# PeterouZh/CIPS-3D

Hardware: AMD Instinct MI355X
Metric: rendered imgs/sec (G fwd+bwd) (higher is better)
Workload: dtype f32 (dense layers as 3-pass split-operand MFMA with fp32 accumulate: SIREN forward on fp16 hi/lo planes, ~2e-7 rel., sigma in the fp32 class; INR head and all backward GEMMs on bf16 hi/lo planes, ~5e-6 rel. per layer; everything else fp32); 1 GPU; FFHQ r64, 24 SIREN evals/ray (num_steps 24, hierarchical False), batch 32/GPU, G fwd+bwd, all 9 CIPS blocks; global_batch=32, parallelism=dp1, rccl_ranks=0, inr_gemm_mode=bf16x3, launch=hipGraph replay, grad_reduce=none

## Files before the change

### cips3d_amd/_lib.py

```python
import ctypes as C
import os

_HERE = os.path.dirname(os.path.abspath(__file__))
LIB_PATH = os.path.join(_HERE, "lib", "libcips3d_hip.so")

vp = C.c_void_p
i32 = C.c_int
i64 = C.c_longlong
f32 = C.c_float


class SirenWeights(C.Structure):
    _fields_ = [(n, vp) for n in
                ("w0", "b0", "w1", "b1", "ws", "bs", "wc", "bc", "wf", "bf",
                 "g0", "p0", "g1", "p1", "gc", "pc")] + [("box_scale", f32), ("trig_mode", i32)]


class SirenGrads(C.Structure):
    _fields_ = [(n, vp) for n in ("dg0", "dp0", "dg1", "dp1", "dgc", "dpc", "dw0", "db0", "dw1", "db1", "dws", "dbs", "dwc",
                                  "dbc", "dwf", "dbf")]


class RayParams(C.Structure):
    _fields_ = [("xg", vp), ("yg", vp), ("zg", vp), ("cam2world", vp), ("jitter", vp), ("zvals", vp), ("zc", f32), ("H", i32),
# ... 120 lines not shown
    "cips_live_points": (i32, [vp, i32, i32, vp, vp, vp]),
    "cips_composite_has_dead_samples": (i32, [i32]),
    "cips_live_points_clamp": (i32, [vp, vp, f32, i32, i32, i32, i32, i32, vp, vp, vp]),
    "cips_composite_bwd_listed": (i32, [vp, vp, vp, vp, f32, vp, vp, vp, i32, i32, i32, i32, vp]),
    "cips_march_fwd_x3_geo": (i32, [C.POINTER(SirenWeights), C.POINTER(RayParams), vp, f32, i32, i32, vp, vp, vp, vp, vp, vp, i32, vp, vp, vp, vp]),
    "cips_composite_fwd_geo": (i32, [vp, vp, vp, vp, vp, vp, vp, f32, vp, vp, vp, vp, vp, i32, i32, i32, i32, vp, vp, vp, vp]),
    "cips_composite_bwd_geo": (i32, [vp, vp, vp, vp, vp, vp, vp, f32, vp, vp, vp, vp, vp, vp, i32, i32, i32, i32, vp, vp, vp, vp]),
    "cips_composite_bwd_live_geo": (i32, [vp, vp, vp, vp, vp, vp, vp, f32, vp, vp, vp, vp, vp, vp, vp, vp, i32, i32, i32, i32, vp, vp, vp, vp]),
    "cips_composite_bwd_listed_geo": (i32, [vp, vp, vp, vp, f32, vp, vp, vp, i32, i32, i32, i32, vp, vp, vp]),
    "cips_gemm_f32": (i32, [C.POINTER(GemmDesc), vp]),
    "cips_gemm_bf16x3": (i32, [C.POINTER(GemmX3Desc), vp]),
    "cips_gemm_bf16x3_fuses_torgb": (i32, [C.POINTER(GemmX3Desc)]),
    "cips_gemm_bf16x3_takes_addp": (i32, [C.POINTER(GemmX3Desc)]),
    "cips_gemm_bf16x3_takes_bkmajor": (i32, [C.POINTER(GemmX3Desc)]),
    "cips_torgb_finish": (i32, [vp, i32, vp, vp, i64, i32, vp]),
    "cips_equal_linear_scratch": (i64, [i32, i32, i32, i32]),
    "cips_equal_linear": (i32, [i32, vp, vp, vp, f32, f32, vp, vp, i32, i32, i32, vp]),
    "cips_gemm_bf16x3_km": (i32, [C.POINTER(GemmX3Desc), vp]),
    "cips_gemm_bf16x3_km_grouped": (i32, [C.POINTER(GemmX3Desc), i32, vp]),
    "cips_gemm_bf16": (i32, [C.POINTER(GemmX3Desc), vp]),
    "cips_gemm_bf16_fuses_torgb": (i32, [C.POINTER(GemmX3Desc)]),
    "cips_gemm_bf16_takes_addp": (i32, [C.POINTER(GemmX3Desc)]),
    "cips_gemm_bf16_km": (i32, [C.POINTER(GemmX3Desc), vp]),
    "cips_gemm_bf16_km_grouped": (i32, [C.POINTER(GemmX3Desc), i32, vp]),
    "cips_lrelu_bwd_bias_slices": (i32, [i32]),
    "cips_lrelu_bwd_bias": (i32, [vp, vp, vp, vp, i64, i32, f32, f32, vp]),
    "cips_lrelu_bwd_bias_finish": (i32, [vp, vp, i32, i32, i32, vp]),
    "cips_lrelu_bwd_bias_nhwc_tiles": (i32, [i32]),
    "cips_lrelu_bwd_bias_nhwc": (i32, [vp, vp, vp, vp, vp, i32, i32, i32, f32, f32, vp]),
    "cips_conv1x1_smallk": (i32, [vp, vp, vp, i32, i32, i32, i32, vp]),
# ... 8 lines not shown
    "cips_conv_weight_prep_max_jobs": (i32, []),
    "cips_conv_weight_prep_batch": (i32, [C.POINTER(WPrepJob), i32, vp]),
    "cips_conv2d_x3_dgrad_s2": (i32, [C.POINTER(ConvDgradS2Desc), vp]),
    "cips_conv_wgrad_finish": (i32, [vp, vp, i32, i32, i32, i32, f32, vp]),
    "cips_conv2d_bf16": (i32, [C.POINTER(ConvX3Desc), vp]),
    "cips_conv2d_bf16_ksplit": (i32, [i32, i32, i32, i32]),
    "cips_conv2d_bf16_dgrad_s2": (i32, [C.POINTER(ConvDgradS2Desc), vp]),
    "cips_conv2d_bf16_wgrad": (i32, [C.POINTER(ConvWgradDesc), vp]),
    "cips_modfc_prep_x3": (i32, [vp, vp, vp, vp, vp, vp, vp, i32, i32, i32, f32, vp]),
    "cips_torgb_fwd_x3": (i32, [vp, vp, vp, vp, vp, i64, i32, i32, vp]),
    "cips_torgb_bwd_w_x3": (i32, [vp, vp, vp, vp, vp, vp, i64, i32, vp]),
    "cips_modfc_prep": (i32, [vp, vp, vp, vp, vp, i32, i32, i32, f32, vp]),
    "cips_modfc_prep_bwd": (i32, [vp, vp, vp, vp, vp, vp, vp, i32, i32, i32, vp]),
    "cips_modfc_max_jobs": (i32, []),
    "cips_modfc_prep_x3_batch": (i32, [C.POINTER(ModfcPrepJob), i32, i32, C.c_float, vp]),
    "cips_modfc_prep_bwd_batch": (i32, [C.POINTER(ModfcBwdJob), i32, i32, vp]),
    "cips_modfc_prep_x3_batch_form": (i32, [C.POINTER(ModfcPrepJob), i32, i32]),
    "cips_modfc_prep_bwd_batch_form": (i32, [C.POINTER(ModfcBwdJob), i32, i32]),
    "cips_modfc_prep_bwd_batch_cores": (i32, [C.POINTER(ModfcBwdJob), i32, i32, vp]),
    "cips_cores_colsum_parts": (i32, []),
    "cips_opt_chunk": (i32, []),
    "cips_opt_step": (i32, [vp, vp, vp, i32, vp, vp, f32, f32, f32, f32, f32, f32, i32, vp, vp]),
    "cips_pyramid_loss_scratch": (i64, [i32, i32, i32, i32, i32]),
    "cips_pyramid_loss_fwd": (i32, [vp, vp, vp, C.POINTER(C.c_double), i32, i32, C.c_double, vp, vp, vp, i64, i32, i32, i32, i32, vp]),
    "cips_pyramid_loss_bwd": (i32, [vp, vp, vp, i32, i64, vp]),
    "cips_reproject_fwd": (i32, [vp, vp, vp, vp, f32, f32, f32, vp, vp, vp, i32, i32, i32, i32, i32, i32, vp]),
    "cips_reproject_bwd": (i32, [vp, vp, vp, vp, vp, f32, f32, vp, vp, i32, i32, i32, i32, i32, i32, vp]),
    "cips_raster_fwd": (i32, [vp] * 5 + [f32, f32, f32, i32] + [vp] * 4 + [i64] + [vp] * 4 + [i32] * 5 + [vp]),
    "cips_raster_interp": (i32, [vp] * 4 + [f32, vp] + [i32] * 6 + [vp]),
    "cips_volume_bake": (i32, [vp] * 4 + [i32] * 4 + [vp]),
# ... 5 lines not shown
    "cips_volume_render_bwd_cam": (i32, [vp] * 8 + [f32, i32, i32] + [vp] * 5 + [i32] * 8 + [vp]),
    "cips_camera_pose": (i32, [vp, vp, i32, f32, f32, f32, f32, vp, vp, vp, i32, vp]),
    "cips_grouped_linear_max_jobs": (i32, []),
    "cips_grouped_linear_fwd": (i32, [C.POINTER(GlinJob), i32, i32, vp]),
    "cips_grouped_linear_scratch": (i64, [C.POINTER(GlinJob), i32, i32]),
    "cips_grouped_linear_bwd": (i32, [C.POINTER(GlinJob), i32, i32, vp, vp, i64, vp]),
    "cips_rownorm_fwd": (i32, [vp, vp, vp, vp, vp, i32, i32, i32, f32, vp]),
    "cips_rownorm_bwd": (i32, [vp] * 9 + [i32, i32, i32, f32, vp]),
    "cips_torgb_fwd": (i32, [vp, vp, vp, vp, i64, i32, i32, vp]),
    "cips_torgb_bwd_partials": (i32, [i64]),
    "cips_torgb_bwd_w": (i32, [vp, vp, vp, vp, vp, i64, i32, vp]),
    "cips_torgb_bwd_x": (i32, [vp, vp, vp, vp, f32, vp, vp, i64, i32, vp]),
    "cips_torgb_bwd_w_x3_batch": (i32, [vp, vp, i32, vp, vp, vp, vp, i64, i32, vp]),
    "cips_torgb_bwd_w_x3_batch_cores": (i32, [vp, vp, i32, vp, vp, vp, vp, i64, i32, vp]),
    "cips_torgb_bwd_x_x3": (i32, [vp, vp, vp, f32, vp, vp, vp, i64, i32, vp]),
    "cips_fused_bias_act": (i32, [vp, vp, vp, vp, i64, i32, i32, i32, i32, f32, f32, vp]),
    "cips_diffaug": (i32, [vp] * 10 + [i32] * 8 + [vp]),
    "cips_avgpool2": (i32, [vp, vp, i64, i32, i32, i32, vp]),
    "cips_axpby": (i32, [vp, vp, vp, f32, f32, i64, vp]),
    "cips_image_to_u8": (i32, [vp, vp, i32, i32, i32, i32, f32, f32, vp]),
    "cips_upfirdn2d": (i32, [vp, vp, vp] + [i32] * 14 + [vp]),
    "cips_upfirdn2d_form": (i32, [i32] * 13),
    "cips_upfirdn2d_parity": (i32, [vp, C.POINTER(i64 * 4), vp, vp] + [i32] * 7 + [vp]),
    "cips_im2col": (i32, [vp, vp] + [i32] * 8 + [vp]),
    "cips_col2im": (i32, [vp, vp] + [i32] * 8 + [vp]),
}

_lib = None


# ... 24 lines not shown
```

### cips3d_amd/csrc/modfc.hip

```cpp
#include "gemm_x3_common.h"
#include <cstdlib>
#include "../../include/cips3d_hip.h"

namespace {

__global__ __launch_bounds__(256) void modfc_prep_kernel(const float* __restrict__ W, const float* __restrict__ s,
                                                         float* __restrict__ wb, float* __restrict__ wbt,
                                                         float* __restrict__ demod, int in_dim, int out_dim, float eps) {
  __shared__ float red[8][33];
  __shared__ float dsh[32];
  const int b = blockIdx.y;
  const int c = threadIdx.x & 31, kg = threadIdx.x >> 5;
  const int n = blockIdx.x * 32 + c;
  const float* sb = s + (long long)b * in_dim;
  float q = 0.f;
  if (n < out_dim)
    for (int k = kg; k < in_dim; k += 8) {
      float u = W[(long long)k * out_dim + n] * (sb[k] + 1.f);
      q = fmaf(u, u, q);
    }
  red[kg][c] = q;
  __syncthreads();
  if (kg == 0) {
    float t = 0.f;
// ... 322 lines not shown
#pragma unroll
      for (int q = 0; q < 8; ++q) v[q] *= ((gb >> q) & 1u) ? 1.f : slope;
    }
    unsigned hw[4], lw[4];
#pragma unroll
    for (int q = 0; q < 4; ++q) {
      const u16 h0 = f2bf(v[2 * q]), h1 = f2bf(v[2 * q + 1]);
      const u16 l0 = f2bf(v[2 * q] - __uint_as_float(((unsigned)h0) << 16)), l1 = f2bf(v[2 * q + 1] - __uint_as_float(((unsigned)h1) << 16));
      hw[q] = (unsigned)h0 | ((unsigned)h1 << 16);
      lw[q] = (unsigned)l0 | ((unsigned)l1 << 16);
    }
    *reinterpret_cast<uint4*>(ph + e) = make_uint4(hw[0], hw[1], hw[2], hw[3]);
    *reinterpret_cast<uint4*>(pl + e) = make_uint4(lw[0], lw[1], lw[2], lw[3]);
  }
}


constexpr int MAXJOBS = 24;
struct PrepJobs {
  const float* W[MAXJOBS]; const float* s[MAXJOBS]; float* demod[MAXJOBS];
  unsigned short *wbh[MAXJOBS], *wbl[MAXJOBS], *wth[MAXJOBS], *wtl[MAXJOBS];
  int in_dim[MAXJOBS], out_dim[MAXJOBS];
};
struct ColJobs {
  const float* W[MAXJOBS]; const float* s[MAXJOBS]; const float* G[MAXJOBS]; float* out[MAXJOBS];
  int in_dim[MAXJOBS], out_dim[MAXJOBS];
};
struct BwdJobs {
  const float* W[MAXJOBS]; const float* s[MAXJOBS]; const float* demod[MAXJOBS]; const float* G[MAXJOBS];
  float *cbuf[MAXJOBS], *dW[MAXJOBS], *ds[MAXJOBS];
// ... 186 lines not shown
      } else {
        const float4 u = make_float4(w.x * m, w.y * m, w.z * m, w.w * m);
        q.x = fmaf(u.x, u.x, q.x); q.y = fmaf(u.y, u.y, q.y); q.z = fmaf(u.z, u.z, q.z); q.w = fmaf(u.w, u.w, q.w);
      }
    }
  }
  red[kg][c] = q;
  __syncthreads();
  if (kg == 0 && n < out_dim) {
    float4 t = make_float4(0.f, 0.f, 0.f, 0.f);
#pragma unroll
    for (int g = 0; g < 16; ++g) { const float4 v = red[g][c]; t.x += v.x; t.y += v.y; t.z += v.z; t.w += v.w; }
    if (WITH_G) *reinterpret_cast<float4*>(J.out[job] + (long long)b * out_dim + n) = t;
    else *reinterpret_cast<float4*>(J.out[job] + (long long)b * out_dim + n) =
        make_float4(rsqrtf(t.x + eps), rsqrtf(t.y + eps), rsqrtf(t.z + eps), rsqrtf(t.w + eps));
  }
}

template <int NCH>
__global__ __launch_bounds__(256) void modfc_prep_bwd_ws_batch_kernel(BwdJobs J, int B) {
  const int job = blockIdx.y;
  const int in_dim = J.in_dim[job], out_dim = J.out_dim[job];
  const int lane = threadIdx.x & 63;
  const int k = blockIdx.x * 4 + (threadIdx.x >> 6);
  if (k >= in_dim) return;
  const float* __restrict__ s = J.s[job]; const float* __restrict__ demod = J.demod[job];
  const float* __restrict__ G = J.G[job]; const float* __restrict__ cbuf = J.cbuf[job];
  float4 w[NCH], acc[NCH];
  bool ok[NCH];
#pragma unroll
// ... 288 lines not shown
    for (int j = 1; j < nblocks; ++j) { const float4 u = part[(long long)j * M + m]; t.x += u.x; t.y += u.y; t.z += u.z; }
    float* o = rgb + m * 3;
    const float r0 = t.x + b0, r1 = t.y + b1, r2 = t.z + b2;
    if (accumulate) { o[0] += r0; o[1] += r1; o[2] += r2; } else { o[0] = r0; o[1] = r1; o[2] = r2; }
  }
}
extern "C" int cips_torgb_finish(const float* part, int nblocks, const float* bias, float* rgb, long long M, int accumulate,
                                 cips_stream_t stream) {
  if (!part || !rgb || nblocks <= 0 || M <= 0 || ((uintptr_t)part & 15)) return (int)hipErrorInvalidValue;
  long long blocks = (M + 255) / 256;
  if (blocks > 4096) blocks = 4096;
  hipLaunchKernelGGL(torgb_finish_kernel, dim3((unsigned)blocks), dim3(256), 0, (hipStream_t)stream,
                     reinterpret_cast<const float4*>(part), nblocks, bias, rgb, M, accumulate);
  return CIPS_CHECK_LAUNCH();
}

extern "C" int cips_torgb_fwd_x3(const void* x_hi, const void* x_lo, const float* w, const float* bias, float* rgb,
                                 long long M, int K, int accumulate, cips_stream_t stream) {
  if (M <= 0 || K <= 0 || (K & 3)) return (int)hipErrorInvalidValue;
  long long blocks = (M + 3) / 4;
  if (blocks > 16384) blocks = 16384;
  if (K == 512) {
    long long b4 = (M + 15) / 16;
    if (b4 > 8192) b4 = 8192;
    hipLaunchKernelGGL(torgb_fwd_x3_k512_kernel, dim3((unsigned)b4), dim3(256), 0, (hipStream_t)stream, (const u16*)x_hi,
                       (const u16*)x_lo, w, bias, rgb, M, accumulate);
    return CIPS_CHECK_LAUNCH();
  }
  hipLaunchKernelGGL(torgb_fwd_kernel<true>, dim3((unsigned)blocks), dim3(256), 0, (hipStream_t)stream, x_hi, x_lo,
                     w, bias, rgb, M, K, accumulate);
// ... 81 lines not shown
  return CIPS_CHECK_LAUNCH();
}


extern "C" int cips_torgb_bwd_x(const float* drgb, const float* w, const float* add, const float* mask,
                                float slope, float* out_unmasked, float* out, long long M, int K,
                                cips_stream_t stream) {
  if (M <= 0 || K <= 0 || (K & 3)) return (int)hipErrorInvalidValue;
  long long blocks = (M * K / 4 + 255) / 256;
  if (blocks > 16384) blocks = 16384;
  hipLaunchKernelGGL(torgb_bwd_x_kernel, dim3((unsigned)blocks), dim3(256), 0, (hipStream_t)stream, drgb, w, add,
                     mask, slope, out_unmasked, out, M, K);
  return CIPS_CHECK_LAUNCH();
}

extern "C" int cips_torgb_bwd_x_x3(const float* drgb, const float* w, const void* gate_bits, float slope, float* out_unmasked,
                                   void* p_hi, void* p_lo, long long M, int K, cips_stream_t stream) {
  if (!drgb || !w || !p_hi || !p_lo || M <= 0 || K <= 0 || (K & 7)) return (int)hipErrorInvalidValue;
  long long blocks = (M * (K / 8) + 255) / 256;
  if (blocks > 16384) blocks = 16384;
  hipLaunchKernelGGL(torgb_bwd_x_x3_kernel, dim3((unsigned)blocks), dim3(256), 0, (hipStream_t)stream, drgb, w,
                     (const unsigned char*)gate_bits, slope, out_unmasked, (u16*)p_hi, (u16*)p_lo, M, K);
  return CIPS_CHECK_LAUNCH();
}

extern "C" int cips_modfc_max_jobs(void) { return MAXJOBS; }

extern "C" int cips_modfc_prep_x3_batch_form(const cips_modfc_prep_job* jobs, int njobs, int B) {
  JobDims D;
  if (const int rc = job_dims(jobs, njobs, B, D)) return -rc;
  return (D.out4 ? CIPS_MODFC_PREP_COLSUM16 : 0)
         | (D.out4 && D.in8 ? CIPS_MODFC_PREP_TILES64 : 0);
}

extern "C" int cips_modfc_prep_bwd_batch_form(const cips_modfc_bwd_job* jobs, int njobs, int B) {
  JobDims D;
  if (const int rc = job_dims(jobs, njobs, B, D)) return -rc;
  if (!(D.out4 && B <= 64 && D.max_out <= 1024)) return CIPS_MODFC_BWD_SCALAR;
  return D.max_out <= 512 ? CIPS_MODFC_BWD_FUSED2 : CIPS_MODFC_BWD_FUSED4;
}

extern "C" int cips_modfc_prep_x3_batch(const cips_modfc_prep_job* jobs, int njobs, int B, float eps, cips_stream_t stream) {
  const int form = cips_modfc_prep_x3_batch_form(jobs, njobs, B);
  if (form < 0) return -form;
  PrepJobs J = {};
  ColJobs Cj = {};
  JobDims D;
  if (const int rc = fill_prep_jobs(jobs, njobs, B, J, Cj, D)) return rc;
  hipStream_t st = (hipStream_t)stream;
  if (form & CIPS_MODFC_PREP_COLSUM16)
    hipLaunchKernelGGL(modfc_colsum4_batch_kernel<false>, dim3((D.max_out + 63) / 64, B, njobs), dim3(256), 0, st, Cj, B, eps);
  else
    hipLaunchKernelGGL(modfc_colsum_batch_kernel<false>, dim3((D.max_out + 31) / 32, B, njobs), dim3(256), 0, st, Cj, eps);
  if (form & CIPS_MODFC_PREP_TILES64)
    hipLaunchKernelGGL(modfc_planes_batch64_kernel, dim3((D.max_out + 63) / 64, (D.max_in + 63) / 64, B * njobs), dim3(256), 0, st, J, B);
  else
    hipLaunchKernelGGL(modfc_planes_batch_kernel, dim3((D.max_out + 31) / 32, (D.max_in + 31) / 32, B * njobs), dim3(256), 0, st, J, B);
  return CIPS_CHECK_LAUNCH();
}

extern "C" int cips_modfc_prep_bwd_batch(const cips_modfc_bwd_job* jobs, int njobs, int B, cips_stream_t stream) {
  const int form = cips_modfc_prep_bwd_batch_form(jobs, njobs, B);
  if (form < 0) return -form;
  BwdJobs J = {};
  ColJobs Cj = {};
  JobDims D;
  if (const int rc = fill_bwd_jobs(jobs, njobs, B, false, J, Cj, D)) return rc;
  hipStream_t st = (hipStream_t)stream;
  if (form == CIPS_MODFC_BWD_SCALAR) return launch_bwd_scalar(J, Cj, D, njobs, B, st);
  hipLaunchKernelGGL(modfc_colsum4_batch_kernel<true>, dim3((D.max_out + 63) / 64, B, njobs), dim3(256), 0, st, Cj, B, 0.f);
  if (form == CIPS_MODFC_BWD_FUSED2)
    hipLaunchKernelGGL(modfc_prep_bwd_ws_batch_kernel<2>, dim3((D.max_in + 3) / 4, njobs), dim3(256), 0, st, J, B);
  else
// ... 4 lines not shown
```

### cips3d_amd/ops.py

```python
import contextlib
import ctypes as C
import math
import os
import weakref
from collections import namedtuple

import torch
from torch.autograd.function import once_differentiable

from . import _lib
from ._lib import (ConvDgradS2Desc, ConvWgradDesc, ConvX3Desc, GemmDesc, GemmX3Desc, GlinJob, GridParams, ModfcBwdJob,
                   ModfcPrepJob, RayParams, SirenGrads, SirenWeights, check)

LRELU_SLOPE = 0.2


def _p(t):
    return C.c_void_p(t.data_ptr()) if t is not None else None


def _stream():
    return C.c_void_p(torch.cuda.current_stream().cuda_stream)


# ... 1058 lines not shown
    check(lib.cips_torgb_fwd(_p(x2d), _p(w), _p(b), _p(rgb2d), M, K, 1 if accumulate else 0, _stream()),
          "cips_torgb_fwd")


def torgb_bwd_w(x2d, drgb2d):
    lib = _lib.load()
    M, K = x2d.shape
    chunks = lib.cips_torgb_bwd_partials(M)
    part = torch.empty(chunks, 4, K, device=x2d.device)
    dw = torch.empty(3, K, device=x2d.device)
    db = torch.empty(3, device=x2d.device)
    check(lib.cips_torgb_bwd_w(_p(x2d), _p(drgb2d), _p(part), _p(dw), _p(db), M, K, _stream()), "cips_torgb_bwd_w")
    return dw, db


def torgb_bwd_x_x3(drgb2d, w, gate_bits, out_unmasked, P):
    lib = _lib.load()
    M, K = drgb2d.shape[0], w.shape[1]
    check(lib.cips_torgb_bwd_x_x3(_p(drgb2d), _p(_c(w)), _p(gate_bits), LRELU_SLOPE, _p(out_unmasked), _p(P.hi), _p(P.lo), M, K,
                                  _stream()), "cips_torgb_bwd_x_x3")


def torgb_bwd_x(drgb2d, w, add, mask, out_unmasked, out):
    lib = _lib.load()
    M = drgb2d.shape[0]
    K = w.shape[1]
    check(lib.cips_torgb_bwd_x(_p(drgb2d), _p(w), _p(add), _p(mask), LRELU_SLOPE, _p(out_unmasked), _p(out), M, K,
                               _stream()), "cips_torgb_bwd_x")


class DebugHook:

    def __init__(self, leftover=None):
        self.pin, self.rec, self.leftover = None, None, leftover

# ... 178 lines not shown

class Planes:
    __slots__ = ("hi", "lo")

    def __init__(self, hi, lo):
        self.hi, self.lo = hi, lo

    @staticmethod
    def empty(*shape, device):
        return Planes(torch.empty(*shape, device=device, dtype=BF), torch.empty(*shape, device=device, dtype=BF))

    def float(self):
        return self.hi.float() + self.lo.float()


X3_KERNEL = 0


def _x3_operands(d, A, Bm, M, N, K, lda, ldb, batch, strideA, strideB, C):
    d.A_hi, d.A_lo, d.B_hi, d.B_lo = _p(A.hi), _p(A.lo), _p(Bm.hi), _p(Bm.lo)
    d.M, d.N, d.K, d.lda, d.ldb = M, N, K, lda, ldb
    d.strideA, d.strideB, d.batch = strideA, strideB, batch
    d.C, d.ldc, d.strideC = _p(C), N, M * N
    d.slope = LRELU_SLOPE
    d.kernel = X3_KERNEL
    return d


def _x3_desc(A, Bm, M, N, K, lda, ldb, batch, strideA, strideB, C=None, P=None, T=None, ldt=0, strideT=0,
             mask_out=None, add=None, rgb_g=None, rgb_w=None, C_unmasked=None, mask=None, act=0, res=None, gate_bits=0,
# ... 50 lines not shown
    ok = _BKMAJOR_OK.get(key)
    if ok is None:
        gq = Planes.empty(1, 8, 8, device=dev)
        epi = {"gate": dict(P=gq, mask=gq.hi, gate_bits=1), "addp": dict(P=gq, mask=gq.hi, gate_bits=1, addp=(gq, gq.hi)),
               "c": dict(C=gq.hi)}[form]
        ok = _BKMAJOR_OK[key] = gemm_x3_takes_bkmajor(gq, gq, n, cin, cout, cout, cin, nb, n * cout, cout * cin, **epi)
    return ok


def gemm_x3(A, Bm, M, N, K, lda, ldb, batch, strideA, strideB, single=False, **epi):
    name, fn = _x3_entry(single)
    d = _x3_desc(A, Bm, M, N, K, lda, ldb, batch, strideA, strideB, **epi)
    check(fn(C.byref(d), _stream()), name)


def gemm_x3_torgb(A, Bm, M, N, K, lda, ldb, batch, strideA, strideB, P, rgb_w, rgb_b, rgb2d, accumulate, single=False, **epi):
    lib = _lib.load()
    name, fn = _x3_entry(single)
    part = torch.empty(max(N // 128, 1), batch * M, 4, device=P.hi.device)
    d = _x3_desc(A, Bm, M, N, K, lda, ldb, batch, strideA, strideB, P=P, torgb=(rgb_w, part), **epi)
    if N % 128 == 0 and rgb_w.is_contiguous() and _x3_entry(single, "_fuses_torgb")[1](C.byref(d)):
        check(fn(C.byref(d), _stream()), name)
        check(lib.cips_torgb_finish(_p(part), N // 128, _p(rgb_b), _p(rgb2d), batch * M, 1 if accumulate else 0, _stream()),
              "cips_torgb_finish")
        return
    d.torgb_w, d.torgb_part = None, None
    check(fn(C.byref(d), _stream()), name)
    torgb_fwd_x3(P, rgb_w, rgb_b, rgb2d, accumulate)


def gemm_x3_km(A, Bm, M, N, K, lda, ldb, batch, strideA, strideB, Cm, single=False):
    name, fn = _x3_entry(single, "_km")
    d = _x3_operands(GemmX3Desc(), A, Bm, M, N, K, lda, ldb, batch, strideA, strideB, Cm)
    check(fn(C.byref(d), _stream()), name)


def gemm_x3_km_grouped(problems, M, N, K, lda, ldb, batch, strideA, strideB, single=False):
    name, fn = _x3_entry(single, "_km_grouped")
    descs = (GemmX3Desc * len(problems))()
    for d, (A, Bm, Cm) in zip(descs, problems):
# ... 196 lines not shown
    in_dim, out_dim = W.shape
    return (Planes.empty(B, in_dim, out_dim, device=W.device) if want_wb else None,
            Planes.empty(B, out_dim, in_dim, device=W.device), torch.empty(B, out_dim, device=W.device))


def modfc_prep_x3(W, s, eps=1e-8, want_wb=True):
    lib = _lib.load()
    in_dim, out_dim = W.shape
    B = s.shape[0]
    wb, wbt, demod = _modfc_prep_x3_out(W, B, want_wb)
    check(lib.cips_modfc_prep_x3(_p(W), _p(s), _p(wb.hi) if wb else None, _p(wb.lo) if wb else None, _p(wbt.hi), _p(wbt.lo),
                                 _p(demod), B, in_dim, out_dim, eps, _stream()), "cips_modfc_prep_x3")
    return wb, wbt, demod


def modfc_prep_x3_batch(layers, eps=1e-8, want_wb=None):
    lib = _lib.load()
    mx = lib.cips_modfc_max_jobs()
    out = []
    for c0 in range(0, len(layers), mx):
        chunk = layers[c0:c0 + mx]
        jobs = (ModfcPrepJob * len(chunk))()
        B = chunk[0][1].shape[0]
        for i, (j, (W, s)) in enumerate(zip(jobs, chunk)):
            wb, wbt, demod = _modfc_prep_x3_out(W, B, want_wb is None or want_wb[c0 + i])
            j.weight, j.s, j.demod = _p(W), _p(s), _p(demod)
            j.wb_hi, j.wb_lo = (_p(wb.hi), _p(wb.lo)) if wb is not None else (None, None)
            j.wbt_hi, j.wbt_lo = _p(wbt.hi), _p(wbt.lo)
            j.in_dim, j.out_dim = W.shape
            out.append((wb, wbt, demod))
        check(lib.cips_modfc_prep_x3_batch(jobs, len(chunk), B, eps, _stream()), "cips_modfc_prep_x3_batch")
    return out


def _modfc_form(entry, job_type, shapes, B):
    jobs = (job_type * max(len(shapes), 1))()
    for j, (in_dim, out_dim) in zip(jobs, shapes):
        j.in_dim, j.out_dim = in_dim, out_dim
    code = getattr(_lib.load(), entry)(jobs, len(shapes), B)
    if code < 0:
        raise ValueError(f"{entry[:-5]} refuses these jobs (hipError {-code})")
    return code


def modfc_prep_x3_batch_form(shapes, B):
    return _modfc_form("cips_modfc_prep_x3_batch_form", ModfcPrepJob, shapes, B)
# ... 187 lines not shown
            L.gate1 = pin1 if pin1 is not None else (torch.empty(B, n, cout // 8, device=dev, dtype=torch.uint8) if bits else L.a1P.hi)
            L.oP = Planes.empty(B, n, cout, device=dev)
            if pin2 is not None:
                L.gate2 = pin2
            elif bits:
                L.gate2 = torch.empty(B, n, cout // 8, device=dev, dtype=torch.uint8)
            elif L.skip:
                L.gate2 = torch.empty(B, n, cout, device=dev, dtype=BF) if train else None
            else:
                L.gate2 = L.oP.hi
            L.wb1, wbt1, L.d1 = prepped[2 * k]
            L.wb2, wbt2, L.d2 = prepped[2 * k + 1]
            L.wbt1, L.wbt2 = (wbt1 if L.wb1 is None else None), (wbt2 if L.wb2 is None else None)
            xP = L.oP
        first_rgb = True
        for k, L in enumerate(layers):
            cin, cout = L.cin, L.cout
            wbt1, wbt2 = prepped[2 * k][1], prepped[2 * k + 1][1]
            res = L.xP if L.skip else None
            if L.pinned1:
                gemm_x3(L.xP, wbt1, n, cout, cin, cin, cin, B, n * cin, cout * cin, P=L.a1P, mask=L.gate1, gate_bits=1, single=sp)
            else:
                gemm_x3(L.xP, wbt1, n, cout, cin, cin, cin, B, n * cin, cout * cin, P=L.a1P, act=1,
                        mask_out=L.gate1 if L.bits else None, gate_bits=2 if L.bits else 0, single=sp)
            mod2 = (L.a1P, wbt2, n, cout, cout, cout, cout, B, n * cout, cout * cout)
            if L.pinned2:
                gemm_x3(*mod2, P=L.oP, res=res, mask=L.gate2, gate_bits=1, single=sp)
            elif L.bits and k >= 3:
                gemm_x3_torgb(*mod2, L.oP, rgbp[2 * (k - 3)], rgbp[2 * (k - 3) + 1], rgb.view(B * n, 3), not first_rgb,
                              act=1, res=res, mask_out=L.gate2, gate_bits=2, single=sp)
                first_rgb = False
                continue
            elif L.bits:
                gemm_x3(*mod2, P=L.oP, act=1, res=res, mask_out=L.gate2, gate_bits=2, single=sp)
            elif L.skip:
                gemm_x3(*mod2, P=L.oP, act=1, res=res, mask_out=L.gate2, single=sp)
            else:
                gemm_x3(*mod2, P=L.oP, act=1, single=sp)
            if k >= 3:
                torgb_fwd_x3(L.oP, rgbp[2 * (k - 3)], rgbp[2 * (k - 3) + 1], rgb.view(B * n, 3), accumulate=not first_rgb)
                first_rgb = False
        if gate_debug.rec is not None:
            for L in layers:
                gate_debug.rec.append(L.gate1)
                gate_debug.rec.append(L.gate2)
        if nblocks <= 3:
            rgb.zero_()
        ctx.layers, ctx.blocks, ctx.rgbp = (layers if train else []), blocks, rgbp
        ctx.dims = (B, n)
        ctx.ports = ports if train else None
        if ctx.ports is not None:
            ports.demod = [d for L in layers for d in (L.d1, L.d2)]
            ports.taps = [L.oP for L in layers[3:]]
        return rgb

    @staticmethod
# ... 628 lines not shown
```

### include/cips3d_hip.h

```cpp
#ifndef CIPS3D_HIP_H
#define CIPS3D_HIP_H

#ifdef __cplusplus
extern "C" {
#endif

typedef void* cips_stream_t;

int cips_version(void);
const char* cips_arch(void);

int cips_rays_fwd(const float* xg, const float* yg, const float* zg, float zc,
                  const float* cam2world, const float* jitter,
                  float* points, float* z, float* dirs,
                  int B, int H, int W, int S, cips_stream_t stream);

typedef struct cips_siren_weights {
  const float* w0;
  const float* b0;
  const float* w1;
  const float* b1;
  const float* ws;
  const float* bs;
  const float* wc;
// ... 214 lines not shown
  int act; float slope;
  const void* res_hi; const void* res_lo;
  int gate_bits;
  const float* torgb_w; float* torgb_part;
  const void* addp_hi; const void* addp_lo; const void* addp_gate; float addp_gain;
  int kernel;
  int b_kmajor;
} cips_gemm_x3_desc;

int cips_gemm_bf16x3(const cips_gemm_x3_desc* d, cips_stream_t stream);
int cips_gemm_bf16x3_takes_bkmajor(const cips_gemm_x3_desc* d);
int cips_gemm_bf16x3_fuses_torgb(const cips_gemm_x3_desc* d);
int cips_gemm_bf16x3_takes_addp(const cips_gemm_x3_desc* d);
int cips_torgb_finish(const float* part, int nblocks, const float* bias, float* rgb, long long M, int accumulate,
                      cips_stream_t stream);
int cips_gemm_bf16x3_km(const cips_gemm_x3_desc* d, cips_stream_t stream);
int cips_gemm_bf16x3_km_grouped(const cips_gemm_x3_desc* descs, int ngroups, cips_stream_t stream);

int cips_gemm_bf16(const cips_gemm_x3_desc* d, cips_stream_t stream);
int cips_gemm_bf16_fuses_torgb(const cips_gemm_x3_desc* d);
int cips_gemm_bf16_takes_addp(const cips_gemm_x3_desc* d);
int cips_gemm_bf16_km(const cips_gemm_x3_desc* d, cips_stream_t stream);
int cips_gemm_bf16_km_grouped(const cips_gemm_x3_desc* descs, int ngroups, cips_stream_t stream);

typedef struct cips_conv_x3_desc {
  const void* w_hi; const void* w_lo;
  const void* x_hi; const void* x_lo;
  float* y;
  int B, C, H, W, O, kh, kw, stride, pad;
  int ksplit;
// ... 52 lines not shown
                        cips_stream_t stream);

typedef struct cips_modfc_prep_job {
  const float* weight; const float* s;
  void *wb_hi, *wb_lo, *wbt_hi, *wbt_lo;
  float* demod;
  int in_dim, out_dim;
} cips_modfc_prep_job;
typedef struct cips_modfc_bwd_job {
  const float* weight; const float* s; const float* demod; const float* gwb;
  float *cbuf, *dweight, *ds;
  int in_dim, out_dim;
} cips_modfc_bwd_job;
int cips_modfc_max_jobs(void);
int cips_modfc_prep_x3_batch(const cips_modfc_prep_job* jobs, int njobs, int B, float eps, cips_stream_t stream);
int cips_modfc_prep_bwd_batch(const cips_modfc_bwd_job* jobs, int njobs, int B, cips_stream_t stream);
enum {
  CIPS_MODFC_PREP_COLSUM16 = 1,
  CIPS_MODFC_PREP_TILES64 = 2
};
enum {
  CIPS_MODFC_BWD_SCALAR = 0,
  CIPS_MODFC_BWD_FUSED2 = 2,
  CIPS_MODFC_BWD_FUSED4 = 4
};
int cips_modfc_prep_x3_batch_form(const cips_modfc_prep_job* jobs, int njobs, int B);
int cips_modfc_prep_bwd_batch_form(const cips_modfc_bwd_job* jobs, int njobs, int B);
int cips_cores_colsum_parts(void);
int cips_modfc_prep_bwd_batch_cores(const cips_modfc_bwd_job* jobs, int njobs, int B, cips_stream_t stream);

// ... 19 lines not shown
int cips_torgb_bwd_partials(long long M);
int cips_torgb_bwd_w(const float* x, const float* drgb, float* partials, float* dw, float* dbias,
                     long long M, int K, cips_stream_t stream);
int cips_torgb_fwd_x3(const void* x_hi, const void* x_lo, const float* w, const float* bias, float* rgb,
                      long long M, int K, int accumulate, cips_stream_t stream);
int cips_torgb_bwd_w_x3(const void* x_hi, const void* x_lo, const float* drgb, float* partials, float* dw,
                        float* dbias, long long M, int K, cips_stream_t stream);
int cips_torgb_bwd_w_x3_batch(const void* const* x_hi, const void* const* x_lo, int njobs, const float* drgb,
                              float* partials, float* dw, float* dbias, long long M, int K, cips_stream_t stream);
int cips_torgb_bwd_w_x3_batch_cores(const void* const* x_hi, const void* const* x_lo, int njobs, const float* drgb,
                                    float* partials, float* dw, float* dbias, long long M, int K, cips_stream_t stream);
int cips_torgb_bwd_x(const float* drgb, const float* w, const float* add, const float* mask, float slope,
                     float* out_unmasked, float* out, long long M, int K, cips_stream_t stream);
int cips_torgb_bwd_x_x3(const float* drgb, const float* w, const void* gate_bits, float slope, float* out_unmasked,
                        void* p_hi, void* p_lo, long long M, int K, cips_stream_t stream);

int cips_camera_pose(const float* theta_raw, const float* phi_raw, int uniform, float h_stddev, float h_mean,
                     float v_stddev, float v_mean, float* pitch_yaw, float* origin, float* cam2world, int B,
                     cips_stream_t stream);

int cips_fused_bias_act(const float* x, const float* bias, const float* refer, float* y,
                        long long numel, int size_b, int step_b,
                        int act, int grad, float alpha, float scale, cips_stream_t stream);

int cips_upfirdn2d(const float* input, const float* kernel, float* out,
                   int major, int in_h, int in_w, int minor, int kernel_h, int kernel_w,
                   int up_x, int up_y, int down_x, int down_y,
                   int pad_x0, int pad_x1, int pad_y0, int pad_y1, cips_stream_t stream);
enum {
  CIPS_UPFIRDN2D_NONE = 0,
// ... 107 lines not shown
```

Measured before the change: 2222 img/s.

## Fuse modfc prep into one kernel, batch torgb finishes, specialize K=512 torgb bwd

Three changes to the INR head. Modulated-FC weight prep now runs as a single strip kernel that computes the demod column sums and writes both weight planes (including a transpose through LDS), replacing the separate colsum and planes launches. The torgb partial-sum finish for several layers is deferred and done by one batched kernel that sums all taps into rgb, instead of one finish launch per layer. The torgb backward-x kernel gets a K=512 variant that keeps the weights in registers and uses one wave per row. Each change is meant to cut launch count and memory passes, at the cost of re-reading W inside the fused prep kernel and possibly lower parallelism.

```diff
diff --git a/cips3d_amd/_lib.py b/cips3d_amd/_lib.py
--- a/cips3d_amd/_lib.py
+++ b/cips3d_amd/_lib.py
@@ -158,6 +158,8 @@
     "cips_gemm_bf16x3_takes_addp": (i32, [C.POINTER(GemmX3Desc)]),
     "cips_gemm_bf16x3_takes_bkmajor": (i32, [C.POINTER(GemmX3Desc)]),
     "cips_torgb_finish": (i32, [vp, i32, vp, vp, i64, i32, vp]),
+    "cips_torgb_finish_max_taps": (i32, []),
+    "cips_torgb_finish_batch": (i32, [vp, vp, i32, i32, vp, i64, i32, vp]),
     "cips_equal_linear_scratch": (i64, [i32, i32, i32, i32]),
     "cips_equal_linear": (i32, [i32, vp, vp, vp, f32, f32, vp, vp, i32, i32, i32, vp]),
     "cips_gemm_bf16x3_km": (i32, [C.POINTER(GemmX3Desc), vp]),
@@ -196,6 +198,7 @@
     "cips_modfc_prep_bwd": (i32, [vp, vp, vp, vp, vp, vp, vp, i32, i32, i32, vp]),
     "cips_modfc_max_jobs": (i32, []),
     "cips_modfc_prep_x3_batch": (i32, [C.POINTER(ModfcPrepJob), i32, i32, C.c_float, vp]),
+    "cips_modfc_prep_x3_batch_two_launch": (i32, [C.POINTER(ModfcPrepJob), i32, i32, C.c_float, vp]),
     "cips_modfc_prep_bwd_batch": (i32, [C.POINTER(ModfcBwdJob), i32, i32, vp]),
     "cips_modfc_prep_x3_batch_form": (i32, [C.POINTER(ModfcPrepJob), i32, i32]),
     "cips_modfc_prep_bwd_batch_form": (i32, [C.POINTER(ModfcBwdJob), i32, i32]),
@@ -231,6 +234,7 @@
     "cips_torgb_bwd_w_x3_batch": (i32, [vp, vp, i32, vp, vp, vp, vp, i64, i32, vp]),
     "cips_torgb_bwd_w_x3_batch_cores": (i32, [vp, vp, i32, vp, vp, vp, vp, i64, i32, vp]),
     "cips_torgb_bwd_x_x3": (i32, [vp, vp, vp, f32, vp, vp, vp, i64, i32, vp]),
+    "cips_torgb_bwd_x_x3_generic": (i32, [vp, vp, vp, f32, vp, vp, vp, i64, i32, vp]),
     "cips_fused_bias_act": (i32, [vp, vp, vp, vp, i64, i32, i32, i32, i32, f32, f32, vp]),
     "cips_diffaug": (i32, [vp] * 10 + [i32] * 8 + [vp]),
     "cips_avgpool2": (i32, [vp, vp, i64, i32, i32, i32, vp]),
diff --git a/cips3d_amd/csrc/modfc.hip b/cips3d_amd/csrc/modfc.hip
--- a/cips3d_amd/csrc/modfc.hip
+++ b/cips3d_amd/csrc/modfc.hip
@@ -360,6 +360,54 @@
     *reinterpret_cast<uint4*>(pl + e) = make_uint4(lw[0], lw[1], lw[2], lw[3]);
   }
 }
+__global__ __launch_bounds__(256) void torgb_bwd_x_x3_k512_kernel(const float* __restrict__ drgb, const float* __restrict__ w,
+                                                                  const unsigned char* __restrict__ gate, float slope,
+                                                                  float* __restrict__ out_unmasked, u16* __restrict__ ph,
+                                                                  u16* __restrict__ pl, long long M) {
+  constexpr int K = 512;
+  const int k = (threadIdx.x & 63) * 8;
+  float4 wr[2][3];
+#pragma unroll
+  for (int h = 0; h < 2; ++h) {
+    wr[h][0] = *reinterpret_cast<const float4*>(w + k + 4 * h);
+    wr[h][1] = *reinterpret_cast<const float4*>(w + K + k + 4 * h);
+    wr[h][2] = *reinterpret_cast<const float4*>(w + 2 * K + k + 4 * h);
+  }
+  const int wave = __builtin_amdgcn_readfirstlane((int)(blockIdx.x * 4 + (threadIdx.x >> 6)));
+  const int nwaves = (int)gridDim.x * 4;
+  for (long long m = wave; m < M; m += nwaves) {
+    const float g0 = drgb[m * 3 + 0], g1 = drgb[m * 3 + 1], g2 = drgb[m * 3 + 2];
+    float v[8];
+#pragma unroll
+    for (int h = 0; h < 2; ++h) {
+      const float4 w0 = wr[h][0], w1 = wr[h][1], w2 = wr[h][2];
+      v[4 * h + 0] = fmaf(g0, w0.x, fmaf(g1, w1.x, g2 * w2.x));
+      v[4 * h + 1] = fmaf(g0, w0.y, fmaf(g1, w1.y, g2 * w2.y));
+      v[4 * h + 2] = fmaf(g0, w0.z, fmaf(g1, w1.z, g2 * w2.z));
+      v[4 * h + 3] = fmaf(g0, w0.w, fmaf(g1, w1.w, g2 * w2.w));
+    }
+    const long long e = m * K + k;
+    if (out_unmasked) {
+      *reinterpret_cast<float4*>(out_unmasked + e) = make_float4(v[0], v[1], v[2], v[3]);
+      *reinterpret_cast<float4*>(out_unmasked + e + 4) = make_float4(v[4], v[5], v[6], v[7]);
+    }
+    if (gate) {
+      const unsigned gb = gate[e >> 3];
+#pragma unroll
+      for (int q = 0; q < 8; ++q) v[q] *= ((gb >> q) & 1u) ? 1.f : slope;
+    }
+    unsigned hw[4], lw[4];
+#pragma unroll
+    for (int q = 0; q < 4; ++q) {
+      const u16 h0 = f2bf(v[2 * q]), h1 = f2bf(v[2 * q + 1]);
+      const u16 l0 = f2bf(v[2 * q] - __uint_as_float(((unsigned)h0) << 16)), l1 = f2bf(v[2 * q + 1] - __uint_as_float(((unsigned)h1) << 16));
+      hw[q] = (unsigned)h0 | ((unsigned)h1 << 16);
+      lw[q] = (unsigned)l0 | ((unsigned)l1 << 16);
+    }
+    *reinterpret_cast<uint4*>(ph + e) = make_uint4(hw[0], hw[1], hw[2], hw[3]);
+    *reinterpret_cast<uint4*>(pl + e) = make_uint4(lw[0], lw[1], lw[2], lw[3]);
+  }
+}
 
 
 constexpr int MAXJOBS = 24;
@@ -576,6 +624,111 @@
     if (WITH_G) *reinterpret_cast<float4*>(J.out[job] + (long long)b * out_dim + n) = t;
     else *reinterpret_cast<float4*>(J.out[job] + (long long)b * out_dim + n) =
         make_float4(rsqrtf(t.x + eps), rsqrtf(t.y + eps), rsqrtf(t.z + eps), rsqrtf(t.w + eps));
+  }
+}
+
+__global__ __launch_bounds__(256, 8) void modfc_prep_strip64_kernel(PrepJobs J, int B, float eps) {
+  __shared__ __attribute__((aligned(16))) unsigned short tile[2][64][64];
+  __shared__ __attribute__((aligned(16))) float dmv[64];
+  float4 (*red)[17] = reinterpret_cast<float4 (*)[17]>(&tile[0][0][0]);
+  const int job = blockIdx.z, b = blockIdx.y;
+  const int in_dim = J.in_dim[job], out_dim = J.out_dim[job];
+  const int n0 = blockIdx.x * 64;
+  if (n0 >= out_dim) return;
+  const float* __restrict__ W = J.W[job];
+  const float* __restrict__ sb = J.s[job] + (long long)b * in_dim;
+  const int t = threadIdx.x;
+  const int c = t & 15, kg = t >> 4;
+  const int n = n0 + 4 * c;
+  const bool nok = n < out_dim;
+  float4 q = make_float4(0.f, 0.f, 0.f, 0.f);
+  if (nok) {
+#pragma unroll 8
+    for (int k = kg; k < in_dim; k += 16) {
+      const float4 w = *reinterpret_cast<const float4*>(W + (long long)k * out_dim + n);
+      const float m = sb[k] + 1.f;
+      const float4 u = make_float4(w.x * m, w.y * m, w.z * m, w.w * m);
+      q.x = fmaf(u.x, u.x, q.x); q.y = fmaf(u.y, u.y, q.y); q.z = fmaf(u.z, u.z, q.z); q.w = fmaf(u.w, u.w, q.w);
+    }
+  }
+  red[kg][c] = q;
+  __syncthreads();
+  if (kg == 0) {
+    float4 d = make_float4(0.f, 0.f, 0.f, 0.f);
+    if (nok) {
+      float4 s4 = make_float4(0.f, 0.f, 0.f, 0.f);
+#pragma unroll 4
+      for (int g = 0; g < 16; ++g) { const float4 v = red[g][c]; s4.x += v.x; s4.y += v.y; s4.z += v.z; s4.w += v.w; }
+      d = make_float4(rsqrtf(s4.x + eps), rsqrtf(s4.y + eps), rsqrtf(s4.z + eps), rsqrtf(s4.w + eps));
+      *reinterpret_cast<float4*>(J.demod[job] + (long long)b * out_dim + n) = d;
+    }
+    *reinterpret_cast<float4*>(&dmv[4 * c]) = d;
+  }
+  __syncthreads();
+  const float4 dm = *reinterpret_cast<const float4*>(&dmv[4 * c]);
+  const bool want_wb = J.wbh[job] != nullptr;
+  const long long base = (long long)b * in_dim * out_dim;
+  unsigned short* __restrict__ wbh = J.wbh[job] + base;
+  unsigned short* __restrict__ wbl = J.wbl[job] + base;
+  unsigned short* __restrict__ wth = J.wth[job] + base;
+  unsigned short* __restrict__ wtl = J.wtl[job] + base;
+  const int c8 = t & 7, r8 = t >> 3;
+  unsigned o_kn = (unsigned)(4 * kg) * out_dim + n;
+  unsigned o_nk = (unsigned)(n0 + r8) * in_dim + 8 * c8;
+  const int piece = 4 * (kg ^ c);
+#pragma unroll 1
+  for (int k0 = 0; k0 < in_dim; k0 += 64) {
+    const bool inside = nok && k0 + 4 * kg < in_dim;
+    float4 wv[4];
+    float sv[4];
+#pragma unroll
+    for (int i = 0; i < 4; ++i) { wv[i] = make_float4(0.f, 0.f, 0.f, 0.f); sv[i] = 0.f; }
+    if (inside) {
+#pragma unroll
+      for (int i = 0; i < 4; ++i) { wv[i] = *reinterpret_cast<const float4*>(W + o_kn + i * out_dim); sv[i] = sb[k0 + 4 * kg + i]; }
+    }
+    unsigned hp[4][2], lp[4][2];
+#pragma unroll
+    for (int i = 0; i < 4; ++i) {
+      const float4 w = wv[i];
+      const float sc = sv[i] + 1.f;
+      const float v[4] = {w.x * sc * dm.x, w.y * sc * dm.y, w.z * sc * dm.z, w.w * sc * dm.w};
+      unsigned short h[4], l[4];
+#pragma unroll
+      for (int j = 0; j < 4; ++j) split_f32(v[j], h[j], l[j]);
+      if (want_wb && inside) {
+        const unsigned o = o_kn + i * out_dim;
+        *reinterpret_cast<uint2*>(wbh + o) = make_uint2((unsigned)h[0] | ((unsigned)h[1] << 16), (unsigned)h[2] | ((unsigned)h[3] << 16));
+        *reinterpret_cast<uint2*>(wbl + o) = make_uint2((unsigned)l[0] | ((unsigned)l[1] << 16), (unsigned)l[2] | ((unsigned)l[3] << 16));
+      }
+#pragma unroll
+      for (int j = 0; j < 4; ++j) {
+        if (i & 1) { hp[j][i >> 1] |= (unsigned)h[j] << 16; lp[j][i >> 1] |= (unsigned)l[j] << 16; }
+        else { hp[j][i >> 1] = h[j]; lp[j][i >> 1] = l[j]; }
+      }
+    }
+    o_kn += 64 * out_dim;
+#pragma unroll
+    for (int j = 0; j < 4; ++j) {
+      *reinterpret_cast<uint2*>(&tile[0][4 * c + j][piece]) = make_uint2(hp[j][0], hp[j][1]);
+      *reinterpret_cast<uint2*>(&tile[1][4 * c + j][piece]) = make_uint2(lp[j][0], lp[j][1]);
+    }
+    __syncthreads();
+#pragma unroll
+    for (int p = 0; p < 2; ++p) {
+      const int nl = r8 + 32 * p;
+      if (n0 + nl < out_dim && k0 + 8 * c8 < in_dim) {
+        const int g = nl >> 2;
+        uint4 xh = *reinterpret_cast<const uint4*>(&tile[0][nl][8 * (c8 ^ (g >> 1))]);
+        uint4 xl = *reinterpret_cast<const uint4*>(&tile[1][nl][8 * (c8 ^ (g >> 1))]);
+        if (g & 1) { xh = make_uint4(xh.z, xh.w, xh.x, xh.y); xl = make_uint4(xl.z, xl.w, xl.x, xl.y); }
+        const unsigned o = o_nk + 32 * p * in_dim;
+        *reinterpret_cast<uint4*>(wth + o) = xh;
+        *reinterpret_cast<uint4*>(wtl + o) = xl;
+      }
+    }
+    o_nk += 64;
+    if (k0 + 64 < in_dim) __syncthreads();
   }
 }
 
@@ -894,6 +1047,43 @@
                      reinterpret_cast<const float4*>(part), nblocks, bias, rgb, M, accumulate);
   return CIPS_CHECK_LAUNCH();
 }
+constexpr int FINISH_MAXTAPS = 8;
+struct FinishTaps { const float4* part[FINISH_MAXTAPS]; const float* bias[FINISH_MAXTAPS]; };
+__global__ __launch_bounds__(256) void torgb_finish_batch_kernel(FinishTaps T, int ntaps, int nblocks, float* __restrict__ rgb,
+                                                                 long long M, int accumulate) {
+  for (long long m = (long long)blockIdx.x * 256 + threadIdx.x; m < M; m += (long long)gridDim.x * 256) {
+    float* o = rgb + m * 3;
+    float a0 = 0.f, a1 = 0.f, a2 = 0.f;
+    if (accumulate) { a0 = o[0]; a1 = o[1]; a2 = o[2]; }
+    for (int i = 0; i < ntaps; ++i) {
+      const float4* __restrict__ part = T.part[i];
+      const float* __restrict__ bias = T.bias[i];
+      const float b0 = bias ? bias[0] : 0.f, b1 = bias ? bias[1] : 0.f, b2 = bias ? bias[2] : 0.f;
+      float4 t = part[m];
+      for (int j = 1; j < nblocks; ++j) { const float4 u = part[(long long)j * M + m]; t.x += u.x; t.y += u.y; t.z += u.z; }
+      const float r0 = t.x + b0, r1 = t.y + b1, r2 = t.z + b2;
+      if (i == 0 && !accumulate) { a0 = r0; a1 = r1; a2 = r2; } else { a0 += r0; a1 += r1; a2 += r2; }
+    }
+    o[0] = a0; o[1] = a1; o[2] = a2;
+  }
+}
+extern "C" int cips_torgb_finish_max_taps(void) { return FINISH_MAXTAPS; }
+extern "C" int cips_torgb_finish_batch(const float* const* parts, const float* const* biases, int ntaps, int nblocks, float* rgb,
+                                       long long M, int accumulate, cips_stream_t stream) {
+  if (!parts || !rgb || ntaps <= 0 || nblocks <= 0 || M <= 0) return (int)hipErrorInvalidValue;
+  if (ntaps > FINISH_MAXTAPS) return (int)hipErrorNotSupported;
+  FinishTaps T = {};
+  for (int i = 0; i < ntaps; ++i) {
+    if (!parts[i] || ((uintptr_t)parts[i] & 15)) return (int)hipErrorInvalidValue;
+    T.part[i] = reinterpret_cast<const float4*>(parts[i]);
+    T.bias[i] = biases ? biases[i] : nullptr;
+  }
+  long long blocks = (M + 255) / 256;
+  if (blocks > 4096) blocks = 4096;
+  hipLaunchKernelGGL(torgb_finish_batch_kernel, dim3((unsigned)blocks), dim3(256), 0, (hipStream_t)stream, T, ntaps, nblocks, rgb,
+                     M, accumulate);
+  return CIPS_CHECK_LAUNCH();
+}
 
 extern "C" int cips_torgb_fwd_x3(const void* x_hi, const void* x_lo, const float* w, const float* bias, float* rgb,
                                  long long M, int K, int accumulate, cips_stream_t stream) {
@@ -1005,14 +1195,32 @@
   return CIPS_CHECK_LAUNCH();
 }
 
-extern "C" int cips_torgb_bwd_x_x3(const float* drgb, const float* w, const void* gate_bits, float slope, float* out_unmasked,
-                                   void* p_hi, void* p_lo, long long M, int K, cips_stream_t stream) {
+namespace {
+int launch_torgb_bwd_x_x3(const float* drgb, const float* w, const void* gate_bits, float slope, float* out_unmasked,
+                          void* p_hi, void* p_lo, long long M, int K, bool generic, cips_stream_t stream) {
   if (!drgb || !w || !p_hi || !p_lo || M <= 0 || K <= 0 || (K & 7)) return (int)hipErrorInvalidValue;
+  if (K == 512 && !generic) {
+    long long b4 = (M + 3) / 4;
+    if (b4 > 2048) b4 = 2048;
+    hipLaunchKernelGGL(torgb_bwd_x_x3_k512_kernel, dim3((unsigned)b4), dim3(256), 0, (hipStream_t)stream, drgb, w,
+                       (const unsigned char*)gate_bits, slope, out_unmasked, (u16*)p_hi, (u16*)p_lo, M);
+    return CIPS_CHECK_LAUNCH();
+  }
   long long blocks = (M * (K / 8) + 255) / 256;
   if (blocks > 16384) blocks = 16384;
   hipLaunchKernelGGL(torgb_bwd_x_x3_kernel, dim3((unsigned)blocks), dim3(256), 0, (hipStream_t)stream, drgb, w,
                      (const unsigned char*)gate_bits, slope, out_unmasked, (u16*)p_hi, (u16*)p_lo, M, K);
   return CIPS_CHECK_LAUNCH();
+}
+}
+
+extern "C" int cips_torgb_bwd_x_x3(const float* drgb, const float* w, const void* gate_bits, float slope, float* out_unmasked,
+                                   void* p_hi, void* p_lo, long long M, int K, cips_stream_t stream) {
+  return launch_torgb_bwd_x_x3(drgb, w, gate_bits, slope, out_unmasked, p_hi, p_lo, M, K, false, stream);
+}
+extern "C" int cips_torgb_bwd_x_x3_generic(const float* drgb, const float* w, const void* gate_bits, float slope,
+                                           float* out_unmasked, void* p_hi, void* p_lo, long long M, int K, cips_stream_t stream) {
+  return launch_torgb_bwd_x_x3(drgb, w, gate_bits, slope, out_unmasked, p_hi, p_lo, M, K, true, stream);
 }
 
 extern "C" int cips_modfc_max_jobs(void) { return MAXJOBS; }
@@ -1031,14 +1239,18 @@
   return D.max_out <= 512 ? CIPS_MODFC_BWD_FUSED2 : CIPS_MODFC_BWD_FUSED4;
 }
 
-extern "C" int cips_modfc_prep_x3_batch(const cips_modfc_prep_job* jobs, int njobs, int B, float eps, cips_stream_t stream) {
+namespace {
+int launch_prep_batch(const cips_modfc_prep_job* jobs, int njobs, int B, float eps, bool one_launch, hipStream_t st) {
   const int form = cips_modfc_prep_x3_batch_form(jobs, njobs, B);
   if (form < 0) return -form;
   PrepJobs J = {};
   ColJobs Cj = {};
   JobDims D;
   if (const int rc = fill_prep_jobs(jobs, njobs, B, J, Cj, D)) return rc;
-  hipStream_t st = (hipStream_t)stream;
+  if (one_launch && form == (CIPS_MODFC_PREP_COLSUM16 | CIPS_MODFC_PREP_TILES64) && D.max_nw < (1LL << 30)) {
+    hipLaunchKernelGGL(modfc_prep_strip64_kernel, dim3((D.max_out + 63) / 64, B, njobs), dim3(256), 0, st, J, B, eps);
+    return CIPS_CHECK_LAUNCH();
+  }
   if (form & CIPS_MODFC_PREP_COLSUM16)
     hipLaunchKernelGGL(modfc_colsum4_batch_kernel<false>, dim3((D.max_out + 63) / 64, B, njobs), dim3(256), 0, st, Cj, B, eps);
   else
@@ -1048,6 +1260,14 @@
   else
     hipLaunchKernelGGL(modfc_planes_batch_kernel, dim3((D.max_out + 31) / 32, (D.max_in + 31) / 32, B * njobs), dim3(256), 0, st, J, B);
   return CIPS_CHECK_LAUNCH();
+}
+}
+
+extern "C" int cips_modfc_prep_x3_batch(const cips_modfc_prep_job* jobs, int njobs, int B, float eps, cips_stream_t stream) {
+  return launch_prep_batch(jobs, njobs, B, eps, true, (hipStream_t)stream);
+}
+extern "C" int cips_modfc_prep_x3_batch_two_launch(const cips_modfc_prep_job* jobs, int njobs, int B, float eps, cips_stream_t stream) {
+  return launch_prep_batch(jobs, njobs, B, eps, false, (hipStream_t)stream);
 }
 
 extern "C" int cips_modfc_prep_bwd_batch(const cips_modfc_bwd_job* jobs, int njobs, int B, cips_stream_t stream) {
diff --git a/cips3d_amd/ops.py b/cips3d_amd/ops.py
--- a/cips3d_amd/ops.py
+++ b/cips3d_amd/ops.py
@@ -1096,11 +1096,11 @@
     return dw, db
 
 
-def torgb_bwd_x_x3(drgb2d, w, gate_bits, out_unmasked, P):
-    lib = _lib.load()
+def torgb_bwd_x_x3(drgb2d, w, gate_bits, out_unmasked, P, generic=False):
+    name = "cips_torgb_bwd_x_x3_generic" if generic or HEAD_LAUNCHES_FORMER else "cips_torgb_bwd_x_x3"
     M, K = drgb2d.shape[0], w.shape[1]
-    check(lib.cips_torgb_bwd_x_x3(_p(drgb2d), _p(_c(w)), _p(gate_bits), LRELU_SLOPE, _p(out_unmasked), _p(P.hi), _p(P.lo), M, K,
-                                  _stream()), "cips_torgb_bwd_x_x3")
+    check(getattr(_lib.load(), name)(_p(drgb2d), _p(_c(w)), _p(gate_bits), LRELU_SLOPE, _p(out_unmasked), _p(P.hi), _p(P.lo), M, K,
+                                     _stream()), name)
 
 
 def torgb_bwd_x(drgb2d, w, add, mask, out_unmasked, out):
@@ -1309,6 +1309,8 @@
         return self.hi.float() + self.lo.float()
 
 
+HEAD_LAUNCHES_FORMER = False
+
 X3_KERNEL = 0
 
 
@@ -1389,16 +1391,45 @@
     check(fn(C.byref(d), _stream()), name)
 
 
-def gemm_x3_torgb(A, Bm, M, N, K, lda, ldb, batch, strideA, strideB, P, rgb_w, rgb_b, rgb2d, accumulate, single=False, **epi):
+class TorgbTaps:
+
+    def __init__(self, rgb2d):
+        self.rgb2d, self.taps, self.accumulate = rgb2d, [], False
+
+    def add(self, part, bias, accumulate):
+        if self.taps and (part.shape != self.taps[0][0].shape or len(self.taps) == _lib.load().cips_torgb_finish_max_taps()):
+            self.flush()
+        if not self.taps:
+            self.accumulate = accumulate
+        self.taps.append((part, bias))
+
+    def flush(self):
+        if not self.taps:
+            return
+        parts = (C.c_void_p * len(self.taps))(*[_p(t[0]) for t in self.taps])
+        biases = (C.c_void_p * len(self.taps))(*[_p(t[1]) for t in self.taps])
+        nblk, M = self.taps[0][0].shape[:2]
+        check(_lib.load().cips_torgb_finish_batch(parts, biases, len(self.taps), nblk, _p(self.rgb2d), M,
+                                                  1 if self.accumulate else 0, _stream()), "cips_torgb_finish_batch")
+        self.taps = []
+
+
+def gemm_x3_torgb(A, Bm, M, N, K, lda, ldb, batch, strideA, strideB, P, rgb_w, rgb_b, rgb2d, accumulate, single=False, taps=None,
+                  **epi):
     lib = _lib.load()
     name, fn = _x3_entry(single)
     part = torch.empty(max(N // 128, 1), batch * M, 4, device=P.hi.device)
     d = _x3_desc(A, Bm, M, N, K, lda, ldb, batch, strideA, strideB, P=P, torgb=(rgb_w, part), **epi)
     if N % 128 == 0 and rgb_w.is_contiguous() and _x3_entry(single, "_fuses_torgb")[1](C.byref(d)):
         check(fn(C.byref(d), _stream()), name)
+        if taps is not None:
+            taps.add(part, rgb_b, accumulate)
+            return
         check(lib.cips_torgb_finish(_p(part), N // 128, _p(rgb_b), _p(rgb2d), batch * M, 1 if accumulate else 0, _stream()),
               "cips_torgb_finish")
         return
+    if taps is not None:
+        taps.flush()
     d.torgb_w, d.torgb_part = None, None
     check(fn(C.byref(d), _stream()), name)
     torgb_fwd_x3(P, rgb_w, rgb_b, rgb2d, accumulate)
@@ -1625,8 +1656,9 @@
     return wb, wbt, demod
 
 
-def modfc_prep_x3_batch(layers, eps=1e-8, want_wb=None):
-    lib = _lib.load()
+def modfc_prep_x3_batch(layers, eps=1e-8, want_wb=None, two_launch=False):
+    lib = _lib.load()
+    name = "cips_modfc_prep_x3_batch_two_launch" if two_launch or HEAD_LAUNCHES_FORMER else "cips_modfc_prep_x3_batch"
     mx = lib.cips_modfc_max_jobs()
     out = []
     for c0 in range(0, len(layers), mx):
@@ -1640,7 +1672,7 @@
             j.wbt_hi, j.wbt_lo = _p(wbt.hi), _p(wbt.lo)
             j.in_dim, j.out_dim = W.shape
             out.append((wb, wbt, demod))
-        check(lib.cips_modfc_prep_x3_batch(jobs, len(chunk), B, eps, _stream()), "cips_modfc_prep_x3_batch")
+        check(getattr(lib, name)(jobs, len(chunk), B, eps, _stream()), name)
     return out
 
 
@@ -1858,6 +1890,7 @@
             L.wbt1, L.wbt2 = (wbt1 if L.wb1 is None else None), (wbt2 if L.wb2 is None else None)
             xP = L.oP
         first_rgb = True
+        taps = None if HEAD_LAUNCHES_FORMER else TorgbTaps(rgb.view(B * n, 3))
         for k, L in enumerate(layers):
             cin, cout = L.cin, L.cout
             wbt1, wbt2 = prepped[2 * k][1], prepped[2 * k + 1][1]
@@ -1872,7 +1905,7 @@
                 gemm_x3(*mod2, P=L.oP, res=res, mask=L.gate2, gate_bits=1, single=sp)
             elif L.bits and k >= 3:
                 gemm_x3_torgb(*mod2, L.oP, rgbp[2 * (k - 3)], rgbp[2 * (k - 3) + 1], rgb.view(B * n, 3), not first_rgb,
-                              act=1, res=res, mask_out=L.gate2, gate_bits=2, single=sp)
+                              act=1, res=res, mask_out=L.gate2, gate_bits=2, single=sp, taps=taps)
                 first_rgb = False
                 continue
             elif L.bits:
@@ -1882,8 +1915,12 @@
             else:
                 gemm_x3(*mod2, P=L.oP, act=1, single=sp)
             if k >= 3:
+                if taps is not None:
+                    taps.flush()
                 torgb_fwd_x3(L.oP, rgbp[2 * (k - 3)], rgbp[2 * (k - 3) + 1], rgb.view(B * n, 3), accumulate=not first_rgb)
                 first_rgb = False
+        if taps is not None:
+            taps.flush()
         if gate_debug.rec is not None:
             for L in layers:
                 gate_debug.rec.append(L.gate1)
diff --git a/include/cips3d_hip.h b/include/cips3d_hip.h
--- a/include/cips3d_hip.h
+++ b/include/cips3d_hip.h
@@ -252,6 +252,9 @@
 int cips_gemm_bf16x3_takes_addp(const cips_gemm_x3_desc* d);
 int cips_torgb_finish(const float* part, int nblocks, const float* bias, float* rgb, long long M, int accumulate,
                       cips_stream_t stream);
+int cips_torgb_finish_max_taps(void);
+int cips_torgb_finish_batch(const float* const* parts, const float* const* biases, int ntaps, int nblocks, float* rgb,
+                            long long M, int accumulate, cips_stream_t stream);
 int cips_gemm_bf16x3_km(const cips_gemm_x3_desc* d, cips_stream_t stream);
 int cips_gemm_bf16x3_km_grouped(const cips_gemm_x3_desc* descs, int ngroups, cips_stream_t stream);
 
@@ -334,6 +337,7 @@
 } cips_modfc_bwd_job;
 int cips_modfc_max_jobs(void);
 int cips_modfc_prep_x3_batch(const cips_modfc_prep_job* jobs, int njobs, int B, float eps, cips_stream_t stream);
+int cips_modfc_prep_x3_batch_two_launch(const cips_modfc_prep_job* jobs, int njobs, int B, float eps, cips_stream_t stream);
 int cips_modfc_prep_bwd_batch(const cips_modfc_bwd_job* jobs, int njobs, int B, cips_stream_t stream);
 enum {
   CIPS_MODFC_PREP_COLSUM16 = 1,
@@ -383,6 +387,8 @@
                      float* out_unmasked, float* out, long long M, int K, cips_stream_t stream);
 int cips_torgb_bwd_x_x3(const float* drgb, const float* w, const void* gate_bits, float slope, float* out_unmasked,
                         void* p_hi, void* p_lo, long long M, int K, cips_stream_t stream);
+int cips_torgb_bwd_x_x3_generic(const float* drgb, const float* w, const void* gate_bits, float slope, float* out_unmasked,
+                                void* p_hi, void* p_lo, long long M, int K, cips_stream_t stream);
 
 int cips_camera_pose(const float* theta_raw, const float* phi_raw, int uniform, float h_stddev, float h_mean,
                      float v_stddev, float v_mean, float* pitch_yaw, float* origin, float* cam2world, int B,
```

New measurement: 2233 img/s (median of 6 runs). Within noise of the previous version (+0.5%).
